# JoeMWatson/input-inference-for-control

Hardware: AMD Instinct MI355X
Metric: i2c timestep-messages/sec (cell-iterations/s = B*T*EM-iters/s), pendulum T=200 B=4096 per GPU (higher is better)
Workload: dtype f64; 1 GPU; pendulum_known_quad cubature i2c (nx=2, nu=1, nz=4), T=200, B=4096 trajectories per GPU, global batch 4096, CubatureQuadrature(1,0,0), alpha0=100, tol=0; batch_per_gpu=4096, horizon=200, parallelism=batch-sharded x1, no collective in the EM loop, kernels=one lane per trajectory

## Files before the change

input-inference-for-control_amd/csrc/i2c_cell.hpp:

```cpp
#pragma once
#include <stdint.h>
#include <type_traits>
#include "../../include/i2c_hip.h"
#include "i2c_linalg.hpp"
#include "i2c_models.hpp"

namespace i2c {

template <typename R> struct Rule {
  R sf;
  R w0;
  R wi;
  R W;
  int unit;
  int gh_degree, gh_points;
  R gh_x[I2C_MAX_GH_DEGREE], gh_w[I2C_MAX_GH_DEGREE];
};

template <class M> struct PerTraj : M {};
template <class M> struct is_per_traj : std::false_type {};
template <class M> struct is_per_traj<PerTraj<M>> : std::true_type {};
template <typename R, bool PER_TRAJ> struct ParamsB {};
template <typename R> struct ParamsB<R, true> {
  const R* params_b;
// ... 91 lines not shown
      M::dynamics(p, xu, sn, cs, y);
    }
  }
};
template <class M, typename R> struct ObserveTermF {
  ParamSrc<M, R> p;
  I2C_HD inline void operator()(const R* x, const R* sn, const R* cs, R* y) const {
    if constexpr (is_per_traj<M>::value) {
      R pb[M::NP];
      M::observe_terminal(param_ptr<M::NP>(p, pb), x, sn, cs, y);
    } else {
      M::observe_terminal(p, x, sn, cs, y);
    }
  }
};

template <class M> struct ObsStruct {
  I2C_HD static constexpr int lin(int k) { return M::obs_lin(k); }
  I2C_HD static constexpr int dep(int k) { return M::obs_dep(k); }
};
template <class M> struct TermStruct {
  I2C_HD static constexpr int lin(int k) { return M::term_lin(k); }
  I2C_HD static constexpr int dep(int k) { return M::term_dep(k); }
};
template <class M> struct MeasStruct {
  I2C_HD static constexpr int lin(int k) { return M::meas_lin(k); }
  I2C_HD static constexpr int dep(int k) { return M::meas_dep(k); }
};
template <int DIN> struct DenseStruct {
  I2C_HD static constexpr int lin(int) { return -1; }
  I2C_HD static constexpr int dep(int) { return DIN - 1; }
};

template <class M, class ST, int DIN, int DOUT, bool CROSS, bool UNITW = false, typename R, class F>
I2C_FN void sp_transform(const Rule<R>& rule, const R* m, const R* Sin, const R* L, const F& f, R* my, R* Sy,
                         R* Sxy, const PolyTab<R>* tab = nullptr) {
  constexpr int NA = M::NA, NA1 = NA > 0 ? NA : 1;
  R s0[NA1], c0[NA1];
#pragma unroll
  for (int a = 0; a < NA; ++a) {
    if (tab)
      r_sincos(m[M::ang(a)], *tab, &s0[a], &c0[a]);
    else
      r_sincos(m[M::ang(a)], &s0[a], &c0[a]);
  }
  R y0[DOUT];
  f(m, s0, c0, y0);
  R A[DOUT];
#pragma unroll
  for (int k = 0; k < DOUT; ++k) A[k] = R(0);
#pragma unroll
  for (int k = 0; k < sym(DOUT); ++k) Sy[k] = R(0);
  if (CROSS) {
#pragma unroll
    for (int k = 0; k < DIN * DOUT; ++k) Sxy[k] = R(0);
  }
#pragma unroll
  for (int j = 0; j < DIN; ++j) {
    bool any = false;
#pragma unroll
    for (int k = 0; k < DOUT; ++k) any = any || (ST::lin(k) < 0 && ST::dep(k) >= j);
    R a[DOUT], dl[DOUT];
    if (any) {
      R xp[DIN], xm[DIN];
#pragma unroll
      for (int i = 0; i < DIN; ++i) {
        if (i < j) {
          xp[i] = m[i];
          xm[i] = m[i];
        } else {
          const R d = rule.sf * L[tri(i, j)];
          xp[i] = m[i] + d;
          xm[i] = m[i] - d;
        }
      }
      R sp[NA1], cp[NA1], sm[NA1], cm[NA1];
#pragma unroll
      for (int q = 0; q < NA; ++q) {
        if (M::ang(q) < j) {
          sp[q] = sm[q] = s0[q];
          cp[q] = cm[q] = c0[q];
        } else {
          R sd, cd;
          if (tab)
            r_sincos(rule.sf * L[tri(M::ang(q), j)], *tab, &sd, &cd);
          else
            r_sincos_small(rule.sf * L[tri(M::ang(q), j)], &sd, &cd);
          sp[q] = s0[q] * cd + c0[q] * sd;
          cp[q] = c0[q] * cd - s0[q] * sd;
          sm[q] = s0[q] * cd - c0[q] * sd;
          cm[q] = c0[q] * cd + s0[q] * sd;
        }
      }
      R yp[DOUT], ym[DOUT];
      f(xp, sp, cp, yp);
      f(xm, sm, cm, ym);
#pragma unroll
      for (int k = 0; k < DOUT; ++k) {
        a[k] = (yp[k] - y0[k]) + (ym[k] - y0[k]);
        dl[k] = yp[k] - ym[k];
      }
    }
#pragma unroll
    for (int k = 0; k < DOUT; ++k) {
      const bool nl_k = ST::lin(k) < 0 && ST::dep(k) >= j;
      if (ST::lin(k) >= j) dl[k] = R(2) * rule.sf * L[tri(ST::lin(k) >= j ? ST::lin(k) : j, j)];
      if (nl_k) A[k] += a[k];
#pragma unroll
      for (int l = 0; l <= k; ++l) {
        const bool nl_l = ST::lin(l) < 0 && ST::dep(l) >= j;
        const bool d_k = nl_k || ST::lin(k) >= j, d_l = nl_l || ST::lin(l) >= j;
        const bool both_lin = ST::lin(k) >= 0 && ST::lin(l) >= 0;
        if (nl_k && nl_l) Sy[tri(k, l)] += a[k] * a[l];
        if (d_k && d_l && !both_lin) Sy[tri(k, l)] += dl[k] * dl[l];
      }
      if (CROSS && nl_k) {
#pragma unroll
        for (int i = j; i < DIN; ++i) Sxy[i * DOUT + k] += L[tri(i, j)] * dl[k];
      }
    }
    sched_fence<(DIN >= 6)>();
  }
  const R hw = R(0.5) * rule.wi, w2 = rule.wi * rule.wi, cs = rule.wi * rule.sf;
#pragma unroll
  for (int k = 0; k < DOUT; ++k) {
    const R Wk = UNITW ? R(1) : rule.W;
    my[k] = ST::lin(k) >= 0 ? Wk * m[ST::lin(k) >= 0 ? ST::lin(k) : 0] : Wk * y0[k] + rule.wi * A[k];
#pragma unroll
    for (int l = 0; l <= k; ++l) {
      if (ST::lin(k) >= 0 && ST::lin(l) >= 0)
        Sy[tri(k, l)] = Sin[tri_any(ST::lin(k) >= 0 ? ST::lin(k) : 0, ST::lin(l) >= 0 ? ST::lin(l) : 0)];
      else
        Sy[tri(k, l)] = hw * Sy[tri(k, l)] - w2 * A[k] * A[l];
    }
    if (CROSS) {
#pragma unroll
      for (int i = 0; i < DIN; ++i)
        Sxy[i * DOUT + k] = ST::lin(k) >= 0 ? Sin[tri_any(i, ST::lin(k) >= 0 ? ST::lin(k) : 0)] : cs * Sxy[i * DOUT + k];
    }
  }
  if (!UNITW && !rule.unit) {
    const R omw = R(1) - rule.W;
    R yc[DOUT];
#pragma unroll
    for (int k = 0; k < DOUT; ++k) yc[k] = ST::lin(k) >= 0 ? m[ST::lin(k) >= 0 ? ST::lin(k) : 0] : y0[k];
#pragma unroll
    for (int k = 0; k < DOUT; ++k)
#pragma unroll
      for (int l = 0; l <= k; ++l)
        Sy[tri(k, l)] += omw * (rule.W * yc[k] * yc[l] + rule.wi * (A[k] * yc[l] + yc[k] * A[l]));
  }
}

template <int DX, int DZ, typename R>
I2C_FN bool kalman_update(R* mu, R* S, const R* mz, R* Sz, R* Sxz, const R* zt) {
  R rinv[DZ];
  const bool ok = chol<DZ>(Sz, rinv);
  R q[DZ];
#pragma unroll
  for (int k = 0; k < DZ; ++k) q[k] = zt[k] - mz[k];
  fsub<DZ>(Sz, rinv, q);
#pragma unroll
  for (int i = 0; i < DX; ++i) {
    fsub<DZ>(Sz, rinv, &Sxz[i * DZ]);
    R v = mu[i];
#pragma unroll
    for (int k = 0; k < DZ; ++k) v += Sxz[i * DZ + k] * q[k];
    mu[i] = v;
// ... 254 lines not shown
  for (int k = 0; k < DOUT; ++k)
#pragma unroll
    for (int l = 0; l <= k; ++l) Sy[tri(k, l)] -= s1[k] * s1[l];
}

constexpr int GRID_LANE = 1, GRID_WAVE = 2;
#ifdef I2C_HOST_SIM
struct GridLaneSim {
  int l;
  double* xch;
};
inline thread_local GridLaneSim grid_lane_sim{0, nullptr};
inline void grid_sim_sync();
#endif
I2C_FN int grid_lane() {
#ifdef I2C_HOST_SIM
  return grid_lane_sim.l;
#else
  return (int)__builtin_amdgcn_mbcnt_hi(~0u, __builtin_amdgcn_mbcnt_lo(~0u, 0u));
#endif
}
template <int GRID> I2C_FN bool grid_writer() {
  if constexpr (GRID == GRID_WAVE) return grid_lane() == 0;
  else return true;
}
template <int GRID> I2C_FN void grid_read_before_write() {
#ifdef I2C_HOST_SIM
  if constexpr (GRID == GRID_WAVE) grid_sim_sync();
#endif
}
template <class M, int DIN, int DOUT, bool CROSS, typename R, class F>
I2C_FN void grid_transform_wave(const Rule<R>& rule, const R* m, const R* L, const F& f, R* my, R* Sy, R* Sxy);

template <int GRID, class M, class ST, int DIN, int DOUT, bool CROSS, bool UNITW = false, typename R, class F>
I2C_FN void transform(const Rule<R>& rule, const R* m, const R* Sin, const R* L, const F& f, R* my, R* Sy, R* Sxy,
                      const PolyTab<R>* tab = nullptr) {
  if constexpr (GRID == GRID_WAVE) {
    grid_transform_wave<M, DIN, DOUT, CROSS>(rule, m, L, f, my, Sy, Sxy);
  } else if constexpr (GRID != 0) {
    if constexpr (DIN <= 3) {
      if (rule.gh_degree == 3) return grid_transform_ct<M, 3, DIN, DOUT, CROSS>(rule, m, L, f, my, Sy, Sxy);
      if (rule.gh_degree == 4) return grid_transform_ct<M, 4, DIN, DOUT, CROSS>(rule, m, L, f, my, Sy, Sxy);
      if (rule.gh_degree == 2) return grid_transform_ct<M, 2, DIN, DOUT, CROSS>(rule, m, L, f, my, Sy, Sxy);
    }
    grid_transform<M, DIN, DOUT, CROSS>(rule, m, L, f, my, Sy, Sxy);
  } else
    sp_transform<M, ST, DIN, DOUT, CROSS, UNITW>(rule, m, Sin, L, f, my, Sy, Sxy, tab);
}


template <typename R, typename S = R> struct FwdArgs {
  const S* prior;
  S* fwd;
  S* prior_out;
  const R* x0;
  const R* sig_x0;
  const R* z;
  const R* alpha;
  const R* alpha_cell;
  const uint8_t* ff;
  int32_t* status;
  const uint8_t* expert;
};

struct NoRelease {
  static constexpr bool ON = false;
  int chunk_len;
  I2C_HD inline void release() const {}
  I2C_HD inline void release_if(int, int) const {}
};
struct ChunkRelease {
  static constexpr bool ON = true;
  int chunk_len;
  I2C_HD inline void release() const {
#if defined(__HIP_DEVICE_COMPILE__)
    __builtin_amdgcn_fence(__ATOMIC_RELEASE, "workgroup");
    __builtin_amdgcn_s_waitcnt(0x0F70);
    __builtin_amdgcn_s_barrier();
#endif
  }
  I2C_HD inline void release_if(const int t, const int at) const {
#if defined(__HIP_DEVICE_COMPILE__)
    asm volatile("s_cmp_lg_u32 %0, %1\n\ts_cbranch_scc1 .Lnot_released_%=\n\ts_waitcnt vmcnt(0)\n\ts_barrier\n.Lnot_released_%=:"
                 :
                 : "s"(t), "s"(at)
                 : "memory", "scc");
#else
    (void)t, (void)at;
#endif
  }
};

template <class M, typename R, bool LEAN = false, int GRID = 0, typename ST_ = R, class REL = NoRelease>
I2C_HD inline void forward_sweep_body(const Consts<M, R>& c, const FwdArgs<R, ST_>& a, const int b, const REL rel = REL{0}) {
  using C = Consts<M, R>;
  constexpr int NX = C::NX, NU = C::NU, NZ = C::NZ, NZT = C::NZT, D = C::D;
  constexpr unsigned W = sizeof(ST_);
  const unsigned long B = c.B;
  const int T = c.T;
  const unsigned bo = (unsigned)b * W;
  const unsigned rb0 = (unsigned)(B * W);
  const R alpha_traj = a.alpha[b];
  const bool wr = grid_writer<GRID>();
  int fail = 0;

  R mu_x[NX], sig_x[sym(NX)];
#pragma unroll
  for (int i = 0; i < NX; ++i) mu_x[i] = a.x0[i * B + b];
#pragma unroll
  for (int i = 0; i < sym(NX); ++i) sig_x[i] = a.sig_x0[i * B + b];

  constexpr bool VOFF = C::D <= 5;
  unsigned voff[VOFF ? C::E_FWD : 1];
  if (VOFF) {
#pragma unroll
    for (int e = 0; e < C::E_FWD; ++e) voff[e] = bo + (unsigned)e * rb0;
  }
  constexpr bool PREFETCH = C::D <= 5;
  R pri[C::E_PRI], zt[NZ];
  if (PREFETCH) {
    const unsigned rb = rb0;
    const Window w = make_window(a.prior + (unsigned long)(LEAN ? 0 : c.row(0)) * C::E_POST * B, (unsigned long)C::E_POST * rb);
#pragma unroll
// ... 145 lines not shown
    {
      R Lf[STRUCT_L0 ? 1 : sym(D)], rinv[D];
      if (!STRUCT_L0) {
#pragma unroll
        for (int i = 0; i < sym(D); ++i) Lf[i] = S0[i];
        cell_bad = flag_stage(cell_bad, chol<D>(Lf, rinv), 1);
      }
      const R* L = STRUCT_L0 ? L0 : Lf;
      R mz[NZ], Sz[sym(NZ)], Sxz[D * NZ];
      transform<GRID, M, ObsStruct<M>, D, NZ, true, LEAN>(c.rule_xu, mu0, S0, L, ObserveF<M, R>{params_of(c, b)}, mz, Sz, Sxz, tab);
#pragma unroll
      for (int i = 0; i < sym(NZ); ++i) Sz[i] += alpha * (CONST_V ? xi0_v[i] : c.sig_xi0[i + kz]);
      cell_bad = flag_stage(cell_bad, kalman_update<D, NZ>(mu0, S0, mz, Sz, Sxz, zt), 2);
    }
    if (!LEAN && PREFETCH && c.z_per_cell) {
#pragma unroll
      for (int k = 0; k < NZ; ++k) zt[k] = a.z[((long)tnr * NZ + k) * B + b];
    }
    const Window out = make_window(a.fwd + (unsigned long)t * C::E_FWD * B, (unsigned long)C::E_FWD * rb);
    if (wr) {
#pragma unroll
      for (int e = 0; e < D; ++e) wst(out, VOFF ? 0u : (e) * rb, VOFF ? voff[e] : bo, (ST_)mu0[e]);
#pragma unroll
      for (int e = 0; e < sym(D); ++e) wst(out, VOFF ? 0u : (D + e) * rb, VOFF ? voff[D + e] : bo, (ST_)S0[e]);
    }

    sched_fence<(D >= 6)>();
    R Sxy[D * NX];
    {
      R L[sym(D)], rinv[D];
#pragma unroll
      for (int i = 0; i < sym(D); ++i) L[i] = S0[i];
      cell_bad = flag_stage(cell_bad, chol<D>(L, rinv), 3);
      transform<GRID, M, DenseStruct<D>, D, NX, true, LEAN>(c.rule_xu, mu0, S0, L, DynamicsF<M, R>{params_of(c, b)}, mu_x, sig_x, Sxy, tab);
    }
#pragma unroll
    for (int i = 0; i < sym(NX); ++i) sig_x[i] += CONST_V ? eta_v[i] : (LEAN ? c.sig_eta[i + kz] : c.sig_eta_w[i + kz]);
    R L3[sym(NX)], rinv3[NX];
#pragma unroll
    for (int i = 0; i < sym(NX); ++i) L3[i] = sig_x[i];
    cell_bad = flag_stage(cell_bad, chol<NX>(L3, rinv3), 4);
    sched_fence<(D >= 6)>();
#pragma unroll
    for (int i = 0; i < D; ++i) {
      fsub<NX>(L3, rinv3, &Sxy[i * NX]);
      bsub<NX>(L3, rinv3, &Sxy[i * NX]);
      sched_fence<(D >= 6)>();
    }

    ff_cur = opaque(ff_cur);
    if (!LEAN) {
      alpha_cur = opaque(alpha_cur);
      if (PREFETCH) {
#pragma unroll
        for (int k = 0; k < NZ; ++k) zt[k] = opaque(zt[k]);
      }
    }
    if (PREFETCH) {
#pragma unroll
      for (int e = 0; e < C::E_PRI; ++e) pri[e] = opaque(pri[e]);
    }
    if constexpr (REL::ON) {
      rel.release_if(t, next_release);
      next_release += t == next_release ? rel.chunk_len : 0;
    }
    if (wr) {
#pragma unroll
      for (int e = 0; e < D * NX; ++e) wst(out, VOFF ? 0u : (D + sym(D) + NX + sym(NX) + e) * rb, VOFF ? voff[D + sym(D) + NX + sym(NX) + e] : bo, (ST_)Sxy[e]);
    }
    sched_fence<(D >= 6)>();

    if (NZT > 0 && t == c.terminal_cell && c.has_Qf) {
      constexpr int NT = C::NZT1;
      R mzt[NT], Szt[sym(NT)], Sxzt[NX * NT];
      transform<GRID, M, TermStruct<M>, NX, NT, true, LEAN>(c.rule_x, mu_x, sig_x, L3, ObserveTermF<M, R>{params_of(c, b)}, mzt, Szt, Sxzt);
#pragma unroll
      for (int i = 0; i < sym(NT); ++i) Szt[i] += alpha * c.sig_xiT0[i];
      cell_bad = flag_stage(cell_bad, kalman_update<NX, NT>(mu_x, sig_x, mzt, Szt, Sxzt, c.zg_term), 5);
      if (STRUCT_L0) {
#pragma unroll
        for (int i = 0; i < sym(NX); ++i) L3[i] = sig_x[i];
        cell_bad = flag_stage(cell_bad, chol<NX>(L3, rinv3), 5);
      }
    }
    if (STRUCT_L0) {
#pragma unroll
      for (int i = 0; i < sym(NX); ++i) Lx[i] = L3[i];
    }
    fail = fold_cell_failure(fail, cell_bad, t);
    if (wr) {
#pragma unroll
      for (int e = 0; e < NX; ++e) wst(out, VOFF ? 0u : (D + sym(D) + e) * rb, VOFF ? voff[D + sym(D) + e] : bo, (ST_)mu_x[e]);
#pragma unroll
      for (int e = 0; e < sym(NX); ++e) wst(out, VOFF ? 0u : (D + sym(D) + NX + e) * rb, VOFF ? voff[D + sym(D) + NX + e] : bo, (ST_)sig_x[e]);
    }

  }
  if constexpr (REL::ON) rel.release();
  if (wr && fail != 0 && a.status[b] == 0) a.status[b] = fail;
}


template <class M, typename R, int GRID = 0>
I2C_FN void end_of_chain(const Consts<M, R>& c, R* temp, const int b, const R* m3f, const R* S3f, R* m3m, R* S3m,
                         int32_t* status) {
  constexpr int NX = M::NX;
  const bool wr = grid_writer<GRID>();
// ... 518 lines not shown
#pragma unroll
    for (int i = 0; i < NX; ++i) {
      R v = mu1[i];
#pragma unroll
      for (int k = 0; k < NX; ++k) v += Jx[i * NX + k] * (av[k] - m3f[k]);
      an[i] = v;
    }
#pragma unroll
    for (int i = 0; i < sym(NX); ++i) Cc[i] = S1[i];
    add_JDJt<NX, NX>(Jx, S3n, Cc);
#pragma unroll
    for (int i = 0; i < NX; ++i)
#pragma unroll
      for (int j = 0; j < NX; ++j) {
        R v = R(0);
#pragma unroll
        for (int k = 0; k < NX; ++k) v += Jx[i * NX + k] * G[k * NX + j];
        Gn[i * NX + j] = v;
      }
#pragma unroll
    for (int i = 0; i < NX; ++i) av[i] = an[i];
#pragma unroll
    for (int i = 0; i < NX * NX; ++i) G[i] = Gn[i];
    cur = nxt;
  }
  constexpr int EC = NX + NX * NX + sym(NX);
  R* out = a.comp + ((long)ch * EC) * B + b;
#pragma unroll
  for (int i = 0; i < NX; ++i) out[(long)i * B] = av[i];
#pragma unroll
  for (int i = 0; i < NX * NX; ++i) out[(long)(NX + i) * B] = G[i];
#pragma unroll
  for (int i = 0; i < sym(NX); ++i) out[(long)(NX + NX * NX + i) * B] = Cc[i];
}

template <int NX, typename R> I2C_FN void apply_composite(const R* av, const R* G, R* Cc, R* m, R* S) {
  R mn[NX];
#pragma unroll
  for (int i = 0; i < NX; ++i) {
    R v = av[i];
#pragma unroll
    for (int k = 0; k < NX; ++k) v += G[i * NX + k] * m[k];
    mn[i] = v;
  }
  add_JDJt<NX, NX>(G, S, Cc);
#pragma unroll
  for (int i = 0; i < NX; ++i) m[i] = mn[i];
#pragma unroll
  for (int i = 0; i < sym(NX); ++i) S[i] = Cc[i];
}

template <class M, typename R, typename S_ = R, int GRID = 0>
I2C_HD inline void chunk_stitch_body(const Consts<M, R>& c, const ChunkArgs<R, S_>& a, const int b) {
  using C = Consts<M, R>;
  constexpr int NX = C::NX, D = C::D;
  constexpr int O_MU3 = D + sym(D), O_S3 = O_MU3 + NX, EC = NX + NX * NX + sym(NX);
  const long B = c.B;
  const S_* last = a.cell.fwd + ((long)(c.T - 1) * C::E_FWD) * B + b;
  R m3f[NX], S3f[sym(NX)], m[NX], S[sym(NX)];
#pragma unroll
  for (int i = 0; i < NX; ++i) m3f[i] = last[(long)(O_MU3 + i) * B];
#pragma unroll
  for (int i = 0; i < sym(NX); ++i) S3f[i] = last[(long)(O_S3 + i) * B];
  end_of_chain<M, R>(c, a.cell.temp, b, m3f, S3f, m, S, a.cell.status);
  terminal_obs_stats<M, R, GRID>(c, b, m, S, a.cell.term_stats, a.cell.status);
  R av[NX], G[NX * NX], Cc[sym(NX)], nav[NX], nG[NX * NX], nCc[sym(NX)];
// ... 689 lines not shown
```

input-inference-for-control_amd/csrc/i2c_impl.hpp:

```cpp
#pragma once
#include "i2c_entry.hpp"
#include "i2c_cell.hpp"
#include "i2c_group.hpp"
#include "i2c_wave.hpp"
#include "i2c_quad.hpp"
#include "i2c_grid.hpp"
#include "i2c_linearize.hpp"

#include <cmath>
#include <cstdio>
#include <cstdlib>
#include <cstring>

namespace i2c {

constexpr int SWEEP_BLOCK = 64;
#ifndef I2C_LANE_BLOCK
#define I2C_LANE_BLOCK 64
#endif
constexpr int LANE_BLOCK = I2C_LANE_BLOCK;
constexpr int CELL_BLOCK = 256;

#ifdef I2C_HOST_SIM
#define I2C_KERNEL(BLOCK) static void
// ... 224 lines not shown
    for (int i = 0; i < 2 * P; ++i) {
      const long t = t0 + i < nc ? t0 + i : nc - 1;
      pm_t[i] = pm.part[(t * 2 + 0) * B + b];
      pv_t[i] = pm.part[(t * 2 + 1) * B + b];
    }
#pragma unroll
    for (int i = 0; i < 2 * P; ++i) {
      const bool in = t0 + i < nc;
      sm[i % P] += in ? pm_t[i] : R(0);
      sv[i % P] += in ? pv_t[i] : R(0);
    }
  }
  R m = R(0), v = R(0);
#pragma unroll
  for (int q = 0; q < P; ++q) {
    m += sm[q];
    v += sv[q];
  }
  pm.term_stats[B + b] = m;
  pm.term_stats[2 * B + b] = v;
  Consts<M, R> cm = c;
  cm.tol = pm.tol;
  mstep_update<M, R>(cm, pm.ms, b, trT, m, v, m, alpha);
}
template <class M, typename R, bool LEAN, typename S = R>
I2C_KERNEL(LANE_BLOCK) k_forward_mstep(I2C_LANE_PARAMS const Consts<M, R> c, const FwdArgs<R, S> a, const int block, const PendingMstep<R> pm) {
  const long b = I2C_LANE_X(block);
  if (b < c.B) {
    finish_pending_mstep<M, R>(c, pm, (int)b);
    forward_sweep_body<M, R, LEAN, 0, S>(c, a, (int)b);
  }
}

template <class M, typename R, bool LEAN, typename S, bool MSTEP>
I2C_FN void forward_helper_lane(const Consts<M, R>& c, const FwdArgs<R, S>& a, const ChunkArgs<R, S>& ch, const PendingMstep<R>& pm,
                                const int role, const int b) {
  if (role == 0) {
    if constexpr (MSTEP) finish_pending_mstep<M, R>(c, pm, b);
    forward_sweep_body<M, R, LEAN, 0, S, ChunkRelease>(c, a, b, ChunkRelease{ch.chunk_len});
  } else {
    for (int k = 0; k < ch.n_chunks; ++k) {
#if defined(__HIP_DEVICE_COMPILE__)
      __builtin_amdgcn_s_barrier();
      __builtin_amdgcn_fence(__ATOMIC_ACQUIRE, "workgroup");
#endif
      chunk_compose_body<M, R, S>(c, ch, k, b);
    }
  }
}
#ifdef I2C_HOST_SIM
constexpr int HELPER_WAVES = 1;
#define I2C_HELPER_LANES                                                                \
  const long b = I2C_LANE_X(LANE_BLOCK);                                                \
  for (int role = 0; role < 2; ++role)
#else
constexpr int HELPER_WAVES = 2;
#define I2C_HELPER_LANES                                                                \
  const long b = (long)blockIdx.x * LANE_BLOCK + (threadIdx.x & (LANE_BLOCK - 1));      \
  const int role = __builtin_amdgcn_readfirstlane((int)(threadIdx.x / LANE_BLOCK));     \
  if (b < c.B)
#endif
template <class M, typename R, bool LEAN, typename S = R>
I2C_KERNEL(2 * LANE_BLOCK) k_forward_helper(I2C_LANE_PARAMS const Consts<M, R> c, const FwdArgs<R, S> a, const ChunkArgs<R, S> ch) {
  I2C_HELPER_LANES forward_helper_lane<M, R, LEAN, S, false>(c, a, ch, PendingMstep<R>{}, role, (int)b);
}
template <class M, typename R, bool LEAN, typename S = R>
I2C_KERNEL(2 * LANE_BLOCK) k_forward_mstep_helper(I2C_LANE_PARAMS const Consts<M, R> c, const FwdArgs<R, S> a, const ChunkArgs<R, S> ch,
                                                  const PendingMstep<R> pm) {
  I2C_HELPER_LANES forward_helper_lane<M, R, LEAN, S, true>(c, a, ch, pm, role, (int)b);
}
#undef I2C_HELPER_LANES


template <typename R> static bool unit_rule(const Rule<R>& r) { return r.unit && r.w0 == R(0); }
template <class M, typename R> static bool unit_rule(const Consts<M, R>& c) { return unit_rule(c.rule_xu) && unit_rule(c.rule_x); }

#ifdef I2C_HOST_SIM
template <typename R, class Body>
static void sim_teams(const int team, const long n_teams, const int n_rows, const bool rows_on_team, const size_t lds, const Body& body) {
  for (int y0 = 0; y0 < (rows_on_team ? 1 : n_rows); ++y0)
    for (long i = 0; i < n_teams; ++i) {
      std::vector<R> sh(lds, R(0)), xch(128, R(0));
      HostBarrier bar(team);
      std::vector<std::thread> lanes;
      for (int l = 0; l < team; ++l)
        lanes.emplace_back([&, l] {
          for (int y = y0; y < (rows_on_team ? n_rows : y0 + 1); ++y) body(i, y, l, lds ? sh.data() : (R*)nullptr, &bar, xch.data());
        });
      for (auto& th : lanes) th.join();
    }
}
#else
template <class M, typename R> __device__ __forceinline__ const Consts<M, R>* kernarg_consts() {
  return (const Consts<M, R>*)__builtin_amdgcn_kernarg_segment_ptr();
}
template <class M, typename R> __device__ __forceinline__ const R* kernarg_zeta() {
  constexpr size_t zoff = (sizeof(Consts<M, R>) + alignof(ZetaArg<M, R>) - 1) / alignof(ZetaArg<M, R>) * alignof(ZetaArg<M, R>);
  return ((const ZetaArg<M, R>*)((const char*)__builtin_amdgcn_kernarg_segment_ptr() + zoff))->v;
}
__device__ __forceinline__ long xcd_first_traj(const unsigned i) {
  const unsigned x = i & 7u, r = (i >> 3) & 3u, g = i >> 5;
  return 16L * (g * 8u + x) + 4 * r;
// ... 462 lines not shown
static bool plan_trace() {
  const char* e = getenv("I2C_TRACE_PLAN");
  return e && atoi(e) == 1;
}
template <class M> struct ChunkWork {
  size_t bnd, part, total;
  ChunkWork(const int B, const int n_chunks) {
    constexpr int NX = M::NX;
    const size_t n = (size_t)n_chunks * (size_t)B;
    bnd = n * (NX + NX * NX + sym(NX));
    part = bnd + n * (NX + sym(NX));
    total = part + n * 3;
  }
};
template <class M> static size_t workspace_elems(int B, int T) {
  int nc, len;
  chunk_geometry(B, T, &nc, &len);
  return ChunkWork<M>(B, nc).total;
}
template <class M, typename R, typename S> static ChunkArgs<R, S> chunk_args(const I2cProblem* p, const CellArgs<R, S>& a) {
  ChunkArgs<R, S> ch{a, (R*)p->work, nullptr, nullptr, 0, 0};
  chunk_geometry(p->B, p->T, &ch.n_chunks, &ch.chunk_len);
  const ChunkWork<M> w(p->B, ch.n_chunks);
  ch.bnd = ch.comp + w.bnd;
  ch.part = ch.comp + w.part;
  return ch;
}

#define I2C_MODEL_CONST(name, MEMBER, DEFAULT)                                                                      \
  template <class M, class = void> struct name : std::integral_constant<int, (DEFAULT)> {};                         \
  template <class M> struct name<M, std::void_t<decltype(M::MEMBER)>> : std::integral_constant<int, M::MEMBER> {};
I2C_MODEL_CONST(bwd_fused_min_b, BWD_FUSED_MIN_B, I2C_BWD_FUSED_MIN_B)
I2C_MODEL_CONST(forward_helper_min_b, FORWARD_HELPER_MIN_B, 4096)
I2C_MODEL_CONST(quad_backward_min_b, QUAD_BACKWARD8_MIN_B, 0)
I2C_MODEL_CONST(quad_backward_max_b, QUAD_BACKWARD8_MAX_B, -1)
I2C_MODEL_CONST(quad_chunk_walk_min_b, QUAD_CHUNK_WALK_MIN_B, 0)
I2C_MODEL_CONST(quad_chunk_walk_max_b, QUAD_CHUNK_WALK_MAX_B, -1)
I2C_MODEL_CONST(quad_chunk_passes_min_b, QUAD_CHUNK_PASSES_MIN_B, 0)
I2C_MODEL_CONST(quad_chunk_passes_max_b, QUAD_CHUNK_PASSES_MAX_B, -1)
I2C_MODEL_CONST(quad_chunk_stitch_max_b, QUAD_CHUNK_STITCH_MAX_B, -1)
#undef I2C_MODEL_CONST


struct Plan {
  int forward, backward, propagate, filter;
  int schedule;
  int walker;
  int compose, stitch;
  int rule;
  bool fwd_tm;
  bool fusable;
};
struct Launches {
  const int schedule;
  const bool self_stitch;
  const bool helper;
  const bool defer;
  const bool reduces;
  const bool walk_lean;
};

template <class M, typename R, typename S = R> struct Impl {
  using C = Consts<M, R>;
  static constexpr bool MIXED = sizeof(S) != sizeof(R);
  static constexpr int G = M::GROUP;
  static constexpr bool HAS_GROUP = G > 0 && sizeof(R) == 8 && !MIXED;
  static constexpr bool LANE = !M::GROUP_ONLY;
  static constexpr bool HAS_WAVE = M::WAVE && sizeof(R) == 8;
  static constexpr bool HAS_QUAD = M::QUAD && sizeof(R) == 8;
  static constexpr bool WIDE = QG<M>::WIDE;
  static constexpr bool HAS_QUAD_BACKWARD = HAS_QUAD && quad_backward_exists<M>();
  static constexpr bool QUAD8 = HAS_QUAD_BACKWARD && !WIDE && LANE;
  static constexpr bool HAS_QUAD_CKF = HAS_QUAD && !MIXED && quad_ckf_exists<M>();
  static constexpr bool HAS_QUAD_PROP = HAS_QUAD && !MIXED && quad_propagate_exists<M>();
  static constexpr bool HAS_GRID = LANE && sizeof(R) == 8 && !MIXED;

  enum Request {
    REQ_DEFAULT,
    REQ_ONE_LANE,
    REQ_GROUP,
    REQ_WAVE,
    REQ_QUAD,
    REQ_QUAD_FORWARD,
    REQ_GRID,
    REQ_NOT_OURS
  };
  static Request request(const int lanes, const int inference) {
    if (lanes == 0) return REQ_DEFAULT;
    if (lanes == -1) return REQ_ONE_LANE;
// ... 209 lines not shown
  static I2cProblem with_unit_rule(const I2cProblem* p) {
    I2cProblem q = *p;
    q.quad_alpha = 1.0, q.quad_beta = 0.0, q.quad_kappa = 0.0;
    return q;
  }
  static C forward_consts(const I2cProblem* p) { return make_consts<M, R>(p, 0.0, p->inference == I2C_INF_LINEARIZE ? p->expert_controller : 0); }
  static C propagate_consts(const I2cProblem* p, const int use_expert) {
    if (p->inference != I2C_INF_LINEARIZE) return make_consts<M, R>(p, 0.0, use_expert);
    const I2cProblem q = with_unit_rule(p);
    return make_consts<M, R>(&q, 0.0, use_expert);
  }
  static C filter_consts(const I2cProblem* p) {
    I2cProblem q = with_unit_rule(p);
    q.inference = I2C_INF_CUBATURE;
    return make_consts<M, R>(&q, 0.0, 0);
  }

  static constexpr bool SELF_STITCH = LANE && C::D <= 5;
  static Launches launches(const I2cProblem* p, const Plan& pl, const C& c, const void* xm, const void* zpost, const void* cell_stats,
                           const bool in_learn) {
    const int mode = schedule_with(pl, p->work != nullptr);
    const bool chunked = mode == I2C_BWD_CHUNKED;
    const bool two_launch = SELF_STITCH && chunked && pl.rule == I2C_INF_CUBATURE && !c.has_x_terminal && !chunk_four_passes();
    const bool self = two_launch && pl.stitch == I2C_FAMILY_LANE && pl.walker == I2C_FAMILY_LANE;
    const bool lane_forward = in_learn && two_launch && pl.forward == I2C_FAMILY_LANE;
    bool helper = lane_forward && pl.compose == I2C_FAMILY_LANE && LANE_BLOCK == 64 && sweep_lanes() == LANE_BLOCK;
    if (helper) {
      const char* e = getenv("I2C_FORWARD_HELPER");
      helper = e ? strcmp(e, "0") != 0 : p->B >= forward_helper_min_b<M>::value;
    }
    const bool reduces = pl.backward == I2C_FAMILY_WAVE   ? mode == I2C_BWD_TWO_PASS && xm && cell_stats
                         : pl.backward == I2C_FAMILY_LANE ? mode != I2C_BWD_FUSED
                                                          : chunked;
    return Launches{mode, self, helper, lane_forward && self, reduces, I2C_WALK_LEAN && !xm && !zpost && !cell_stats && !c.z_per_cell};
  }

  template <bool LEAN>
  static int launch_forward_lane(const I2cProblem* p, const Launches& L, const C& c, const FwdArgs<R, S>& a, const PendingMstep<R>& pend, void* stream) {
    const int lanes = sweep_lanes();
    if constexpr (SELF_STITCH) {
      if (L.helper) {
        constexpr int W = HELPER_WAVES;
        const ChunkArgs<R, S> ch = chunk_args<M>(p, CellArgs<R, S>{a.fwd});
        return pend.part ? launch(k_forward_mstep_helper<M, R, LEAN, S>, W * (long)p->B, 1, W * LANE_BLOCK, stream, c, a, ch, pend)
                         : launch(k_forward_helper<M, R, LEAN, S>, W * (long)p->B, 1, W * LANE_BLOCK, stream, c, a, ch);
      }
      if (pend.part) return launch(k_forward_mstep<M, R, LEAN, S>, p->B, 1, lanes, stream, c, a, lanes, pend);
    }
    return launch(k_forward<M, R, LEAN, false, S>, p->B, 1, lanes, stream, c, a, lanes);
  }
  static int run_forward(const I2cProblem* p, const Plan& pl, const Launches& L, const C& c, const void* prior, void* fwd, void* prior_out,
                         int32_t* status, void* stream, const PendingMstep<R>& pend = {}) {
    if (pl.forward < 0) return pl.forward;
    const FwdArgs<R, S> a{(const S*)prior, (S*)fwd, (S*)prior_out, (const R*)p->x0, (const R*)p->sig_x0,
                          (const R*)p->z,  (const R*)p->alpha, (const R*)p->alpha_cell, p->feedforward, status, p->expert};
    if (pl.forward == I2C_FAMILY_WAVE) {
      if constexpr (HAS_WAVE) return launch_wave<WK_FORWARD, M, R, S>(c, a, stream);
    }
    if (pl.forward == I2C_FAMILY_QUAD) {
      if constexpr (HAS_QUAD) {
        C cq = c;
        cq.fwd_tm = pl.fwd_tm;
        return launch_quad_forward<M, R, S>(cq, a, stream);
      }
    }
    if (pl.forward == I2C_FAMILY_GROUP) {
      if constexpr (HAS_GROUP) return launch_group<GK_FORWARD, M, R, G>(c, nullptr, a, stream);
    }
    if (pl.forward == I2C_FAMILY_GRID) {
      if constexpr (HAS_GRID) return launch_grid<GRK_FORWARD, M, R>(c, a, stream);
    }
    if constexpr (LANE) {
      if constexpr (!MIXED) {
        if (pl.rule == I2C_INF_LINEARIZE) return launch(k_forward_lin<M, R>, p->B, 1, LANE_BLOCK, stream, c, a);
        if (pl.rule == I2C_INF_GAUSS_HERMITE) return launch(k_forward<M, R, false, true>, p->B, 1, LANE_BLOCK, stream, c, a, LANE_BLOCK);
      }
      const bool lean = c.rule_xu.unit && c.rule_x.unit && !c.z_per_cell && !a.alpha_cell && !a.prior_out && c.t0 == 0;
      if (plan_trace()) fprintf(stderr, "i2c_forward_lane: sweep=%s lean=%d\n", L.helper ? "helper" : "plain", (int)lean);
      return lean ? launch_forward_lane<true>(p, L, c, a, pend, stream) : launch_forward_lane<false>(p, L, c, a, pend, stream);
    }
    return I2C_ENOTSUP;
  }
  static int forward(const I2cProblem* p, const void* prior, void* fwd, void* prior_out, int32_t* status, void* stream) {
    const Plan pl = resolve(p);
    const C c = forward_consts(p);
    return run_forward(p, pl, launches(p, pl, c, nullptr, nullptr, nullptr, false), c, prior, fwd, prior_out, status, stream);
  }

  static const R* terminal_alpha(const I2cProblem* p, const C& c) {
    return p->alpha_cell ? (const R*)p->alpha_cell + (long)c.row(p->T - 1) * (long)p->B : (const R*)p->alpha;
  }
  static MstepArgs<R> mstep_args(const I2cProblem* p, const void* term_stats, void* stats_out, const int update = 1) {
    return MstepArgs<R>{(const R*)term_stats, (R*)p->alpha, (R*)stats_out, update};
  }
  static MstepArgs<R> no_mstep(const void* term_stats) { return MstepArgs<R>{(const R*)term_stats, nullptr, nullptr, 0}; }
  static int run_backward(const I2cProblem* p, const Plan& pl, const Launches& L, const C& c, const void* fwd, void* xm, void* post, void* zpost,
                          void* cell_stats, void* term_stats, int32_t* status, void* stream, const MstepArgs<R>& ms, const bool last = true) {
    if (pl.backward < 0) return pl.backward;
    if (pl.schedule < 0) return pl.schedule;
    const CellArgs<R, S> a{(const S*)fwd,  (const S*)xm,   (const R*)p->z, (S*)post, (S*)zpost,
                           (R*)cell_stats, (R*)term_stats, (R*)p->temp,    status,   terminal_alpha(p, c)};
    const int mode = L.schedule;
    int rc = I2C_ENOTSUP;
    if (pl.backward == I2C_FAMILY_WAVE) {
      if constexpr (HAS_WAVE) {
        if (mode != I2C_BWD_TWO_PASS || !a.xm || !a.cell_stats) return launch_wave<WK_BACKWARD, M, R, S>(c, a, stream);
        rc = launch_wave<WK_SCAN, M, R, S>(c, a, stream);
        if (rc == I2C_OK) rc = launch_wave<WK_CELL, M, R, S>(c, a, stream);
        if (rc == I2C_OK) rc = launch_reduce<M, R>(c, a, ms, p->T, stream);
      }
      return rc;
// ... 338 lines not shown
```

Before: 2.419 billion timestep-messages/s.

## Hand off smoother-gain computation from forward sweep lane to helper wave

In the self-stitched forward sweep with a helper wave, the sweep lane now stores raw sigma-point differences instead of forming the cross-covariance and solving for the smoother gain. The helper wave redoes the Cholesky factorisations, builds the gain from those differences, and writes it back while it composes each chunk. This takes work off the serial critical path of the forward sweep and puts it on the helper wave, which was otherwise idle. The cost is repeated Cholesky work, an extra terminal covariance buffer (reusing ch.part), and extra global loads and stores in the helper. It is enabled by default for models with D<=3 and can be overridden with an environment variable.

```diff
diff --git a/input-inference-for-control_amd/csrc/i2c_cell.hpp b/input-inference-for-control_amd/csrc/i2c_cell.hpp
--- a/input-inference-for-control_amd/csrc/i2c_cell.hpp
+++ b/input-inference-for-control_amd/csrc/i2c_cell.hpp
@@ -147,9 +147,11 @@
   I2C_HD static constexpr int dep(int) { return DIN - 1; }
 };
 
-template <class M, class ST, int DIN, int DOUT, bool CROSS, bool UNITW = false, typename R, class F>
+template <class M, class ST, int DIN, int DOUT, bool CROSS, bool UNITW = false, bool HANDOFF = false, typename R, class F>
 I2C_FN void sp_transform(const Rule<R>& rule, const R* m, const R* Sin, const R* L, const F& f, R* my, R* Sy,
                          R* Sxy, const PolyTab<R>* tab = nullptr) {
+  static_assert(!HANDOFF || (CROSS && ST::lin(0) < 0 && ST::dep(0) == DIN - 1 && ST::lin(DOUT - 1) < 0 && ST::dep(DOUT - 1) == DIN - 1),
+                "the hand-off of the differences is the dense callback's");
   constexpr int NA = M::NA, NA1 = NA > 0 ? NA : 1;
   R s0[NA1], c0[NA1];
 #pragma unroll
@@ -166,7 +168,7 @@
   for (int k = 0; k < DOUT; ++k) A[k] = R(0);
 #pragma unroll
   for (int k = 0; k < sym(DOUT); ++k) Sy[k] = R(0);
-  if (CROSS) {
+  if (CROSS && !HANDOFF) {
 #pragma unroll
     for (int k = 0; k < DIN * DOUT; ++k) Sxy[k] = R(0);
   }
@@ -229,7 +231,8 @@
         if (nl_k && nl_l) Sy[tri(k, l)] += a[k] * a[l];
         if (d_k && d_l && !both_lin) Sy[tri(k, l)] += dl[k] * dl[l];
       }
-      if (CROSS && nl_k) {
+      if (CROSS && HANDOFF) Sxy[j * DOUT + k] = dl[k];
+      if (CROSS && !HANDOFF && nl_k) {
 #pragma unroll
         for (int i = j; i < DIN; ++i) Sxy[i * DOUT + k] += L[tri(i, j)] * dl[k];
       }
@@ -248,7 +251,7 @@
       else
         Sy[tri(k, l)] = hw * Sy[tri(k, l)] - w2 * A[k] * A[l];
     }
-    if (CROSS) {
+    if (CROSS && !HANDOFF) {
 #pragma unroll
       for (int i = 0; i < DIN; ++i)
         Sxy[i * DOUT + k] = ST::lin(k) >= 0 ? Sin[tri_any(i, ST::lin(k) >= 0 ? ST::lin(k) : 0)] : cs * Sxy[i * DOUT + k];
@@ -569,9 +572,10 @@
 template <class M, int DIN, int DOUT, bool CROSS, typename R, class F>
 I2C_FN void grid_transform_wave(const Rule<R>& rule, const R* m, const R* L, const F& f, R* my, R* Sy, R* Sxy);
 
-template <int GRID, class M, class ST, int DIN, int DOUT, bool CROSS, bool UNITW = false, typename R, class F>
+template <int GRID, class M, class ST, int DIN, int DOUT, bool CROSS, bool UNITW = false, bool HANDOFF = false, typename R, class F>
 I2C_FN void transform(const Rule<R>& rule, const R* m, const R* Sin, const R* L, const F& f, R* my, R* Sy, R* Sxy,
                       const PolyTab<R>* tab = nullptr) {
+  static_assert(!HANDOFF || GRID == 0, "the hand-off of the differences is the sigma-point rule's (sp_transform)");
   if constexpr (GRID == GRID_WAVE) {
     grid_transform_wave<M, DIN, DOUT, CROSS>(rule, m, L, f, my, Sy, Sxy);
   } else if constexpr (GRID != 0) {
@@ -582,7 +586,7 @@
     }
     grid_transform<M, DIN, DOUT, CROSS>(rule, m, L, f, my, Sy, Sxy);
   } else
-    sp_transform<M, ST, DIN, DOUT, CROSS, UNITW>(rule, m, Sin, L, f, my, Sy, Sxy, tab);
+    sp_transform<M, ST, DIN, DOUT, CROSS, UNITW, HANDOFF>(rule, m, Sin, L, f, my, Sy, Sxy, tab);
 }
 
 
@@ -601,13 +605,13 @@
 };
 
 struct NoRelease {
-  static constexpr bool ON = false;
+  static constexpr bool ON = false, GAIN = false;
   int chunk_len;
   I2C_HD inline void release() const {}
   I2C_HD inline void release_if(int, int) const {}
 };
 struct ChunkRelease {
-  static constexpr bool ON = true;
+  static constexpr bool ON = true, GAIN = false;
   int chunk_len;
   I2C_HD inline void release() const {
 #if defined(__HIP_DEVICE_COMPILE__)
@@ -626,6 +630,13 @@
     (void)t, (void)at;
 #endif
   }
+};
+template <typename R> struct ChunkReleaseGain {
+  static constexpr bool ON = true, GAIN = true;
+  int chunk_len;
+  R* term_sig;
+  I2C_HD inline void release() const { ChunkRelease{chunk_len}.release(); }
+  I2C_HD inline void release_if(const int t, const int at) const { ChunkRelease{chunk_len}.release_if(t, at); }
 };
 
 template <class M, typename R, bool LEAN = false, int GRID = 0, typename ST_ = R, class REL = NoRelease>
@@ -837,7 +848,7 @@
 #pragma unroll
       for (int i = 0; i < sym(D); ++i) L[i] = S0[i];
       cell_bad = flag_stage(cell_bad, chol<D>(L, rinv), 3);
-      transform<GRID, M, DenseStruct<D>, D, NX, true, LEAN>(c.rule_xu, mu0, S0, L, DynamicsF<M, R>{params_of(c, b)}, mu_x, sig_x, Sxy, tab);
+      transform<GRID, M, DenseStruct<D>, D, NX, true, LEAN, REL::GAIN>(c.rule_xu, mu0, S0, L, DynamicsF<M, R>{params_of(c, b)}, mu_x, sig_x, Sxy, tab);
     }
 #pragma unroll
     for (int i = 0; i < sym(NX); ++i) sig_x[i] += CONST_V ? eta_v[i] : (LEAN ? c.sig_eta[i + kz] : c.sig_eta_w[i + kz]);
@@ -846,11 +857,13 @@
     for (int i = 0; i < sym(NX); ++i) L3[i] = sig_x[i];
     cell_bad = flag_stage(cell_bad, chol<NX>(L3, rinv3), 4);
     sched_fence<(D >= 6)>();
-#pragma unroll
-    for (int i = 0; i < D; ++i) {
-      fsub<NX>(L3, rinv3, &Sxy[i * NX]);
-      bsub<NX>(L3, rinv3, &Sxy[i * NX]);
-      sched_fence<(D >= 6)>();
+    if constexpr (!REL::GAIN) {
+#pragma unroll
+      for (int i = 0; i < D; ++i) {
+        fsub<NX>(L3, rinv3, &Sxy[i * NX]);
+        bsub<NX>(L3, rinv3, &Sxy[i * NX]);
+        sched_fence<(D >= 6)>();
+      }
     }
 
     ff_cur = opaque(ff_cur);
@@ -878,6 +891,12 @@
     if (NZT > 0 && t == c.terminal_cell && c.has_Qf) {
       constexpr int NT = C::NZT1;
       R mzt[NT], Szt[sym(NT)], Sxzt[NX * NT];
+      if constexpr (REL::GAIN) {
+        if (wr) {
+#pragma unroll
+          for (int i = 0; i < sym(NX); ++i) rel.term_sig[(unsigned long)i * B + b] = sig_x[i];
+        }
+      }
       transform<GRID, M, TermStruct<M>, NX, NT, true, LEAN>(c.rule_x, mu_x, sig_x, L3, ObserveTermF<M, R>{params_of(c, b)}, mzt, Szt, Sxzt);
 #pragma unroll
       for (int i = 0; i < sym(NT); ++i) Szt[i] += alpha * c.sig_xiT0[i];
@@ -1462,6 +1481,127 @@
   for (int i = 0; i < NX * NX; ++i) out[(long)(NX + i) * B] = G[i];
 #pragma unroll
   for (int i = 0; i < sym(NX); ++i) out[(long)(NX + NX * NX + i) * B] = Cc[i];
+}
+
+template <class M, typename R> I2C_FN void gain_from_handoff(const Rule<R>& rule, const R* S_xu1, const R* S_x3, R* J) {
+  constexpr int NX = M::NX, D = M::NX + M::NU;
+  R L[sym(D)], rinv[D], Sxy[D * NX];
+#pragma unroll
+  for (int i = 0; i < sym(D); ++i) L[i] = S_xu1[i];
+  chol<D>(L, rinv);
+#pragma unroll
+  for (int k = 0; k < D * NX; ++k) Sxy[k] = R(0);
+#pragma unroll
+  for (int j = 0; j < D; ++j)
+#pragma unroll
+    for (int k = 0; k < NX; ++k)
+#pragma unroll
+      for (int i = j; i < D; ++i) Sxy[i * NX + k] += L[tri(i, j)] * J[j * NX + k];
+  const R cs = rule.wi * rule.sf;
+#pragma unroll
+  for (int k = 0; k < NX; ++k)
+#pragma unroll
+    for (int i = 0; i < D; ++i) Sxy[i * NX + k] = cs * Sxy[i * NX + k];
+  R L3[sym(NX)], rinv3[NX];
+#pragma unroll
+  for (int i = 0; i < sym(NX); ++i) L3[i] = S_x3[i];
+  chol<NX>(L3, rinv3);
+#pragma unroll
+  for (int i = 0; i < D; ++i) {
+    fsub<NX>(L3, rinv3, &Sxy[i * NX]);
+    bsub<NX>(L3, rinv3, &Sxy[i * NX]);
+  }
+#pragma unroll
+  for (int k = 0; k < D * NX; ++k) J[k] = Sxy[k];
+}
+
+template <class M, typename R>
+I2C_HD inline void chunk_compose_gain_body(const Consts<M, R>& c, const ChunkArgs<R, R>& a, const R* term_sig, const int ch, const int b) {
+  using C = Consts<M, R>;
+  constexpr int NX = C::NX, D = C::D;
+  constexpr int O_MU3 = D + sym(D), O_S3 = O_MU3 + NX, O_J = O_S3 + sym(NX);
+  const long B = c.B;
+  const int t_lo = ch * a.chunk_len, t_hi = (t_lo + a.chunk_len < c.T) ? t_lo + a.chunk_len : c.T;
+  const int t_term = (C::NZT > 0 && c.has_Qf) ? c.terminal_cell : -1;
+  R av[NX], G[NX * NX], Cc[sym(NX)];
+#pragma unroll
+  for (int i = 0; i < NX; ++i) av[i] = R(0);
+#pragma unroll
+  for (int i = 0; i < NX; ++i)
+#pragma unroll
+    for (int j = 0; j < NX; ++j) G[i * NX + j] = i == j ? R(1) : R(0);
+#pragma unroll
+  for (int i = 0; i < sym(NX); ++i) Cc[i] = R(0);
+  struct Row {
+    R mu1[NX], S1[sym(D)], m3f[NX], S3f[sym(NX)], S3g[sym(NX)], J[D * NX];
+  };
+  auto load = [&](int t, Row& r) {
+    const R* in = a.cell.fwd + ((long)t * C::E_FWD) * B + b;
+    const R* s3 = t == t_term ? term_sig + b : in + (long)O_S3 * B;
+#pragma unroll
+    for (int i = 0; i < NX; ++i) r.mu1[i] = in[(long)i * B];
+#pragma unroll
+    for (int i = 0; i < sym(D); ++i) r.S1[i] = in[(long)(D + i) * B];
+#pragma unroll
+    for (int i = 0; i < NX; ++i) r.m3f[i] = in[(long)(O_MU3 + i) * B];
+#pragma unroll
+    for (int i = 0; i < sym(NX); ++i) r.S3f[i] = in[(long)(O_S3 + i) * B];
+#pragma unroll
+    for (int i = 0; i < sym(NX); ++i) r.S3g[i] = s3[(long)i * B];
+#pragma unroll
+    for (int i = 0; i < D * NX; ++i) r.J[i] = in[(long)(O_J + i) * B];
+  };
+  Row cur, nxt;
+  load(t_hi - 1, cur);
+  for (int t = t_hi - 1; t >= t_lo; --t) {
+    load(t > t_lo ? t - 1 : t_lo, nxt);
+    gain_from_handoff<M, R>(c.rule_xu, cur.S1, cur.S3g, cur.J);
+    R* out = const_cast<R*>(a.cell.fwd) + ((long)t * C::E_FWD + O_J) * B + b;
+#pragma unroll
+    for (int i = 0; i < D * NX; ++i) out[(long)i * B] = cur.J[i];
+    R Jx[NX * NX];
+#pragma unroll
+    for (int i = 0; i < NX * NX; ++i) Jx[i] = opaque(cur.J[i]);
+    const R* mu1 = cur.mu1;
+    const R* S1 = cur.S1;
+    const R* m3f = cur.m3f;
+    R S3n[sym(NX)];
+#pragma unroll
+    for (int i = 0; i < sym(NX); ++i) S3n[i] = Cc[i] - cur.S3f[i];
+    R an[NX], Gn[NX * NX];
+#pragma unroll
+    for (int i = 0; i < NX; ++i) {
+      R v = mu1[i];
+#pragma unroll
+      for (int k = 0; k < NX; ++k) v += Jx[i * NX + k] * (av[k] - m3f[k]);
+      an[i] = v;
+    }
+#pragma unroll
+    for (int i = 0; i < sym(NX); ++i) Cc[i] = S1[i];
+    add_JDJt<NX, NX>(Jx, S3n, Cc);
+#pragma unroll
+    for (int i = 0; i < NX; ++i)
+#pragma unroll
+      for (int j = 0; j < NX; ++j) {
+        R v = R(0);
+#pragma unroll
+        for (int k = 0; k < NX; ++k) v += Jx[i * NX + k] * G[k * NX + j];
+        Gn[i * NX + j] = v;
+      }
+#pragma unroll
+    for (int i = 0; i < NX; ++i) av[i] = an[i];
+#pragma unroll
+    for (int i = 0; i < NX * NX; ++i) G[i] = Gn[i];
+    cur = nxt;
+  }
+  constexpr int EC = NX + NX * NX + sym(NX);
+  R* comp = a.comp + ((long)ch * EC) * B + b;
+#pragma unroll
+  for (int i = 0; i < NX; ++i) comp[(long)i * B] = av[i];
+#pragma unroll
+  for (int i = 0; i < NX * NX; ++i) comp[(long)(NX + i) * B] = G[i];
+#pragma unroll
+  for (int i = 0; i < sym(NX); ++i) comp[(long)(NX + NX * NX + i) * B] = Cc[i];
 }
 
 template <int NX, typename R> I2C_FN void apply_composite(const R* av, const R* G, R* Cc, R* m, R* S) {
diff --git a/input-inference-for-control_amd/csrc/i2c_impl.hpp b/input-inference-for-control_amd/csrc/i2c_impl.hpp
--- a/input-inference-for-control_amd/csrc/i2c_impl.hpp
+++ b/input-inference-for-control_amd/csrc/i2c_impl.hpp
@@ -280,10 +280,25 @@
   }
 }
 
-template <class M, typename R, bool LEAN, typename S, bool MSTEP>
+template <class M, typename R, bool LEAN, typename S, bool MSTEP, bool GAINH>
 I2C_FN void forward_helper_lane(const Consts<M, R>& c, const FwdArgs<R, S>& a, const ChunkArgs<R, S>& ch, const PendingMstep<R>& pm,
                                 const int role, const int b) {
-  if (role == 0) {
+  if constexpr (GAINH) {
+    static_assert(sizeof(S) == sizeof(R), "the gain hand-off is not rounded to a narrower storage type");
+    R* const term_sig = ch.part;
+    if (role == 0) {
+      if constexpr (MSTEP) finish_pending_mstep<M, R>(c, pm, b);
+      forward_sweep_body<M, R, LEAN, 0, S, ChunkReleaseGain<R>>(c, a, b, ChunkReleaseGain<R>{ch.chunk_len, term_sig});
+    } else {
+      for (int k = 0; k < ch.n_chunks; ++k) {
+#if defined(__HIP_DEVICE_COMPILE__)
+        __builtin_amdgcn_s_barrier();
+        __builtin_amdgcn_fence(__ATOMIC_ACQUIRE, "workgroup");
+#endif
+        chunk_compose_gain_body<M, R>(c, ch, term_sig, k, b);
+      }
+    }
+  } else if (role == 0) {
     if constexpr (MSTEP) finish_pending_mstep<M, R>(c, pm, b);
     forward_sweep_body<M, R, LEAN, 0, S, ChunkRelease>(c, a, b, ChunkRelease{ch.chunk_len});
   } else {
@@ -308,14 +323,14 @@
   const int role = __builtin_amdgcn_readfirstlane((int)(threadIdx.x / LANE_BLOCK));     \
   if (b < c.B)
 #endif
-template <class M, typename R, bool LEAN, typename S = R>
+template <class M, typename R, bool LEAN, typename S = R, bool GAINH = false>
 I2C_KERNEL(2 * LANE_BLOCK) k_forward_helper(I2C_LANE_PARAMS const Consts<M, R> c, const FwdArgs<R, S> a, const ChunkArgs<R, S> ch) {
-  I2C_HELPER_LANES forward_helper_lane<M, R, LEAN, S, false>(c, a, ch, PendingMstep<R>{}, role, (int)b);
-}
-template <class M, typename R, bool LEAN, typename S = R>
+  I2C_HELPER_LANES forward_helper_lane<M, R, LEAN, S, false, GAINH>(c, a, ch, PendingMstep<R>{}, role, (int)b);
+}
+template <class M, typename R, bool LEAN, typename S = R, bool GAINH = false>
 I2C_KERNEL(2 * LANE_BLOCK) k_forward_mstep_helper(I2C_LANE_PARAMS const Consts<M, R> c, const FwdArgs<R, S> a, const ChunkArgs<R, S> ch,
                                                   const PendingMstep<R> pm) {
-  I2C_HELPER_LANES forward_helper_lane<M, R, LEAN, S, true>(c, a, ch, pm, role, (int)b);
+  I2C_HELPER_LANES forward_helper_lane<M, R, LEAN, S, true, GAINH>(c, a, ch, pm, role, (int)b);
 }
 #undef I2C_HELPER_LANES
 
@@ -844,6 +859,7 @@
   template <class M> struct name<M, std::void_t<decltype(M::MEMBER)>> : std::integral_constant<int, M::MEMBER> {};
 I2C_MODEL_CONST(bwd_fused_min_b, BWD_FUSED_MIN_B, I2C_BWD_FUSED_MIN_B)
 I2C_MODEL_CONST(forward_helper_min_b, FORWARD_HELPER_MIN_B, 4096)
+I2C_MODEL_CONST(forward_helper_gain, FORWARD_HELPER_GAIN, M::NX + M::NU <= 3)
 I2C_MODEL_CONST(quad_backward_min_b, QUAD_BACKWARD8_MIN_B, 0)
 I2C_MODEL_CONST(quad_backward_max_b, QUAD_BACKWARD8_MAX_B, -1)
 I2C_MODEL_CONST(quad_chunk_walk_min_b, QUAD_CHUNK_WALK_MIN_B, 0)
@@ -867,6 +883,7 @@
   const int schedule;
   const bool self_stitch;
   const bool helper;
+  const bool helper_gain;
   const bool defer;
   const bool reduces;
   const bool walk_lean;
@@ -1142,7 +1159,11 @@
     const bool reduces = pl.backward == I2C_FAMILY_WAVE   ? mode == I2C_BWD_TWO_PASS && xm && cell_stats
                          : pl.backward == I2C_FAMILY_LANE ? mode != I2C_BWD_FUSED
                                                           : chunked;
-    return Launches{mode, self, helper, lane_forward && self, reduces, I2C_WALK_LEAN && !xm && !zpost && !cell_stats && !c.z_per_cell};
+    const char* const eg = getenv("I2C_FORWARD_HELPER_GAIN");
+    int n_chunks, chunk_len;
+    chunk_geometry(p->B, p->T, &n_chunks, &chunk_len);
+    const bool helper_gain = helper && !MIXED && 3 * n_chunks >= sym(C::NX) && (eg ? strcmp(eg, "0") != 0 : forward_helper_gain<M>::value != 0);
+    return Launches{mode, self, helper, helper_gain, lane_forward && self, reduces, I2C_WALK_LEAN && !xm && !zpost && !cell_stats && !c.z_per_cell};
   }
 
   template <bool LEAN>
@@ -1152,6 +1173,11 @@
       if (L.helper) {
         constexpr int W = HELPER_WAVES;
         const ChunkArgs<R, S> ch = chunk_args<M>(p, CellArgs<R, S>{a.fwd});
+        if constexpr (!MIXED) {
+          if (L.helper_gain)
+            return pend.part ? launch(k_forward_mstep_helper<M, R, LEAN, S, true>, W * (long)p->B, 1, W * LANE_BLOCK, stream, c, a, ch, pend)
+                             : launch(k_forward_helper<M, R, LEAN, S, true>, W * (long)p->B, 1, W * LANE_BLOCK, stream, c, a, ch);
+        }
         return pend.part ? launch(k_forward_mstep_helper<M, R, LEAN, S>, W * (long)p->B, 1, W * LANE_BLOCK, stream, c, a, ch, pend)
                          : launch(k_forward_helper<M, R, LEAN, S>, W * (long)p->B, 1, W * LANE_BLOCK, stream, c, a, ch);
       }
@@ -1186,7 +1212,8 @@
         if (pl.rule == I2C_INF_GAUSS_HERMITE) return launch(k_forward<M, R, false, true>, p->B, 1, LANE_BLOCK, stream, c, a, LANE_BLOCK);
       }
       const bool lean = c.rule_xu.unit && c.rule_x.unit && !c.z_per_cell && !a.alpha_cell && !a.prior_out && c.t0 == 0;
-      if (plan_trace()) fprintf(stderr, "i2c_forward_lane: sweep=%s lean=%d\n", L.helper ? "helper" : "plain", (int)lean);
+      if (plan_trace())
+        fprintf(stderr, "i2c_forward_lane: sweep=%s lean=%d gain=%s\n", L.helper ? "helper" : "plain", (int)lean, L.helper_gain ? "helper" : "sweep");
       return lean ? launch_forward_lane<true>(p, L, c, a, pend, stream) : launch_forward_lane<false>(p, L, c, a, pend, stream);
     }
     return I2C_ENOTSUP;
```

After: 2.497 billion timestep-messages/s (median of 6 runs). 3.2% higher.
